# qope/SIPP

Measured on AMD Instinct MI355X. Metric: SIPP proof-gen wall-clock + pairings-aggregated/sec, n=128 (the 3 STARK sub-proofs, hardened G1/G2 AIRs; outer plonky2 proof not included), higher is better.
Workload: dtype u64; 1 GPU; n=128 SIPP instance per GPU: G1ExpStark 127 IO (N=2^16, W+P+Q=1176), G2ExpStark 127 IO (N=2^16, 2314), Fq12ExpStark 14 IO (N=2^13, 7970); IO records on host -> 3 flat proofs on host, the 3 sub-proofs on 3 concurrent HIP streams; parallelism=1 independent SIPP instance(s), one per GPU, no collective

## Files before the change

### include/sipp_hip.h

```cpp
#ifndef SIPP_HIP_H
#define SIPP_HIP_H

#include <stddef.h>
#include <stdint.h>

#ifdef __cplusplus
extern "C" {
#endif

typedef struct sipp_ctx sipp_ctx;

typedef enum {
    SIPP_OK = 0,
    SIPP_E_BADARG = -1,
    SIPP_E_HIP = -2,
    SIPP_E_NOMEM = -3,
    SIPP_E_BUFSZ = -4,
    SIPP_E_SUBGROUP = -5,
    SIPP_E_QUOTIENT = -6,
    SIPP_E_UNSUPPORTED = -7,
    SIPP_E_WITNESS = -8,
    SIPP_E_VERIFY = -9
} sipp_status;

// ... 48 lines not shown
void *sipp_stream(sipp_ctx *ctx);

int sipp_g1_exp_prove(sipp_ctx *ctx, const uint32_t *ios, size_t num_io, uint64_t *proof_out, size_t proof_cap,
                      size_t *proof_len);
int sipp_g2_exp_prove(sipp_ctx *ctx, const uint32_t *ios, size_t num_io, uint64_t *proof_out, size_t proof_cap,
                      size_t *proof_len);
int sipp_fq12_exp_prove(sipp_ctx *ctx, const uint32_t *ios, size_t num_io, uint64_t *proof_out, size_t proof_cap,
                        size_t *proof_len);
int sipp_prove(sipp_ctx *ctx, int kind, const uint32_t *ios, size_t num_io, uint64_t *proof_out, size_t proof_cap,
               size_t *proof_len);
int sipp_prove_async(sipp_ctx *ctx, int kind, const uint32_t *ios, size_t num_io, uint64_t *proof_out,
                     size_t proof_cap);
int sipp_wait(sipp_ctx *ctx, size_t *proof_len);
int sipp_instance_prove(sipp_ctx *const ctxs[3], const uint32_t *const ios[3], const size_t num_io[3],
                        uint64_t *const proof_out[3], const size_t proof_cap[3], size_t proof_len[3]);
int sipp_instances_prove(sipp_ctx *const *ctxs, size_t in_flight, size_t count, const uint32_t *const *ios,
                         const size_t *num_io, uint64_t *const *proof_out, const size_t *proof_cap, size_t *proof_len,
                         int *status);
int sipp_io_shard(size_t num_io, uint32_t world, uint32_t rank, size_t *first, size_t *count);
int sipp_exp_outputs(sipp_ctx *ctx, int kind, uint32_t *ios, size_t num_io);
size_t sipp_proof_size(const sipp_ctx *ctx, int kind, size_t num_io);
size_t sipp_workspace_bytes(int kind, size_t num_io);
size_t sipp_workspace_bytes_cfg(int kind, size_t num_io, const sipp_stark_config *cfg);
int sipp_device_memory(int device, size_t *free_bytes, size_t *total_bytes);
int sipp_stark_shape(const sipp_ctx *ctx, int kind, size_t num_io, uint32_t *log_rows, uint32_t *main_cols,
                     uint32_t *perm_cols, uint32_t *quotient_cols);

int sipp_map_to_g2_prove(sipp_ctx *ctx, const uint32_t *ios, size_t num_io, uint64_t *proof_out, size_t proof_cap,
                         size_t *proof_len);
int sipp_pairing_prove(sipp_ctx *ctx, const uint32_t *ios, size_t num_io, uint64_t *proof_out, size_t proof_cap,
                       size_t *proof_len);
int sipp_stark_verify(const uint64_t *proof, size_t len, const sipp_stark_config *cfg, int *reason);

int sipp_map_to_g2(sipp_ctx *ctx, const uint32_t *msgs, size_t n, uint32_t *map_ios, uint32_t *g2_ios, uint32_t *cleared);

int sipp_inner_product(sipp_ctx *ctx, const uint32_t *g1, const uint32_t *g2, size_t n, uint32_t *out);
int sipp_inner_products(sipp_ctx *ctx, const uint32_t *g1, const uint32_t *g2, size_t n, size_t count, uint32_t *out);

size_t sipp_native_proof_words(size_t n);
int sipp_prove_native(sipp_ctx *ctx, const uint32_t *A, const uint32_t *B, size_t n, uint32_t *proof);
int sipp_verify_native(sipp_ctx *ctx, const uint32_t *A, const uint32_t *B, size_t n, const uint32_t *proof,
                       uint32_t *statement, uint32_t *g1_ios, uint32_t *g2_ios, uint32_t *fq12_ios, int *accepted);

#define SIPP_SALT_SIZE 4
#define SIPP_FRI_MAX_ROUNDS 32
typedef struct {
// ... 170 lines not shown
```

### rust_shim/src/ffi.rs

```rust
use std::os::raw::{c_char, c_int, c_void};

#[repr(C)]
pub struct SippCtxOpaque {
    _p: [u8; 0],
}

#[repr(C)]
#[derive(Clone, Copy)]
pub struct SippStarkConfig {
    pub rate_bits: u32,
    pub cap_height: u32,
    pub pow_bits: u32,
    pub arity_bits: u32,
    pub final_poly_bits: u32,
    pub num_queries: u32,
    pub num_challenges: u32,
    pub pow_rule: u32,
    pub fs_rule: u32,
    pub lookup_rule: u32,
}

pub const SIPP_G1_EXP: c_int = 0;
pub const SIPP_G2_EXP: c_int = 1;
pub const SIPP_FQ12_EXP: c_int = 2;
// ... 171 lines not shown
    pub fn sipp_circuit_workspace_bytes(log_n: u32, p: *const SippPlonkParams, fp: *const SippFriParams, c: *const SippPlonkCircuit) -> usize;
    pub fn sipp_circuit_build(ctx: *mut SippCtxOpaque, log_n: u32, p: *const SippPlonkParams, fp: *const SippFriParams, c: *const SippPlonkCircuit,
                              constants_sigmas: *const u64, gens: *const SippPlonkGenerator, n_gens: usize, sched: *const SippPlonkScheduleHost,
                              circuit_digest: *const u64, out: *mut *mut SippCircuitDataOpaque) -> c_int;
    pub fn sipp_circuit_destroy(cd: *mut SippCircuitDataOpaque);
    pub fn sipp_circuit_verifier_data(cd: *const SippCircuitDataOpaque, cap_out: *mut u64, digest_out: *mut u64) -> c_int;
    pub fn sipp_circuit_proof_size(cd: *const SippCircuitDataOpaque, n_public_inputs: u32) -> usize;
    pub fn sipp_circuit_prove(cd: *mut SippCircuitDataOpaque, wires: *const u64, public_inputs: *const u64, n_public_inputs: u32,
                              proof_out: *mut u64, proof_cap: usize, proof_len: *mut usize) -> c_int;
    pub fn sipp_circuit_prove_inputs(cd: *mut SippCircuitDataOpaque, cells: *const u64, values: *const u64, n_inputs: usize,
                                     public_inputs: *const u64, n_public_inputs: u32, proof_out: *mut u64, proof_cap: usize,
                                     proof_len: *mut usize) -> c_int;
    pub fn sipp_circuit_set_input_map(cd: *mut SippCircuitDataOpaque, cells: *const u64, sources: *const u64, n: usize, n_words: usize,
                                      n_extra: usize) -> c_int;
    pub fn sipp_circuit_prove_words(cd: *mut SippCircuitDataOpaque, words: *const u64, n_words: usize, extra: *const u64, n_extra: usize,
                                    public_inputs: *const u64, n_public_inputs: u32, proof_out: *mut u64, proof_cap: usize,
                                    proof_len: *mut usize) -> c_int;
    pub fn sipp_circuit_verify(cd: *const SippCircuitDataOpaque, proof: *const u64, len: usize, reason: *mut c_int) -> c_int;
    pub fn sipp_plonk_verify_gates(proof: *const u64, len: usize, constants_sigmas_cap: *const u64, p: *const SippPlonkParams, fp: *const SippFriParams,
                                   c: *const SippPlonkCircuit, circuit_digest: *const u64, reason: *mut c_int) -> c_int;
    pub fn sipp_proof_size(ctx: *const SippCtxOpaque, kind: c_int, num_io: usize) -> usize;
    pub fn sipp_workspace_bytes(kind: c_int, num_io: usize) -> usize;
    pub fn sipp_workspace_bytes_cfg(kind: c_int, num_io: usize, cfg: *const SippStarkConfig) -> usize;
    pub fn sipp_device_memory(device: c_int, free_bytes: *mut usize, total_bytes: *mut usize) -> c_int;
    pub fn sipp_stark_shape(ctx: *const SippCtxOpaque, kind: c_int, num_io: usize, log_rows: *mut u32, main_cols: *mut u32,
                            perm_cols: *mut u32, quotient_cols: *mut u32) -> c_int;
    pub fn sipp_inner_product(ctx: *mut SippCtxOpaque, g1: *const u32, g2: *const u32, n: usize, out: *mut u32) -> c_int;
    pub fn sipp_inner_products(ctx: *mut SippCtxOpaque, g1: *const u32, g2: *const u32, n: usize, count: usize, out: *mut u32) -> c_int;
    pub fn sipp_native_proof_words(n: usize) -> usize;
    pub fn sipp_prove_native(ctx: *mut SippCtxOpaque, A: *const u32, B: *const u32, n: usize, proof: *mut u32) -> c_int;
    pub fn sipp_verify_native(ctx: *mut SippCtxOpaque, A: *const u32, B: *const u32, n: usize, proof: *const u32, statement: *mut u32,
                              g1_ios: *mut u32, g2_ios: *mut u32, fq12_ios: *mut u32, accepted: *mut c_int) -> c_int;
    pub fn sipp_fri_const_arity(p: *mut SippFriParams, arity_bits: u32, final_poly_bits: u32, degree_bits: u32);
    pub fn sipp_commit_batch_ex(ctx: *mut SippCtxOpaque, d_in: *const u64, from_coeffs: c_int, d_coeffs: *mut u64, d_lde: *mut u64,
                                d_tree: *mut u64, ncols: usize, log_n: u32, rate_bits: u32, cap_height: u32, d_salt: *const u64,
                                n_salt: u32, cap_out: *mut u64) -> c_int;
    pub fn sipp_fri_proof_size(oracles: *const SippOracle, n_oracles: usize, batches: *const SippFriBatch, n_batches: usize, log_n: u32,
                               p: *const SippFriParams) -> usize;
    pub fn sipp_fri_prove_openings(ctx: *mut SippCtxOpaque, oracles: *const SippOracle, n_oracles: usize, batches: *const SippFriBatch,
                                   n_batches: usize, log_n: u32, p: *const SippFriParams, ch: *mut SippChallenger, proof_out: *mut u64,
                                   proof_cap: usize, proof_len: *mut usize) -> c_int;
    pub fn sipp_plonk_num_partial_products(p: *const SippPlonkParams) -> u32;
    pub fn sipp_plonk_zs_partial_products(ctx: *mut SippCtxOpaque, d_wires: *const u64, d_sigmas: *const u64, log_n: u32, p: *const SippPlonkParams,
                                          betas: *const u64, gammas: *const u64, d_out: *mut u64) -> c_int;
    pub fn sipp_plonk_quotient_chunks(ctx: *mut SippCtxOpaque, d_wires_lde: *const u64, d_sigmas_lde: *const u64, d_zs_lde: *const u64, log_n: u32,
                                      rate_bits: u32, p: *const SippPlonkParams, betas: *const u64, gammas: *const u64, alphas: *const u64,
// ... 35 lines not shown
```

### sipp_amd/_lib.py

```python
import ctypes as C
import json
import os

import numpy as np

HERE = os.path.dirname(os.path.abspath(__file__))
SO = os.path.join(HERE, "libsipp_hip.so")

P = 2**64 - 2**32 + 1

STATUS = {
    0: "SIPP_OK", -1: "SIPP_E_BADARG", -2: "SIPP_E_HIP", -3: "SIPP_E_NOMEM", -4: "SIPP_E_BUFSZ",
    -5: "SIPP_E_SUBGROUP", -6: "SIPP_E_QUOTIENT", -7: "SIPP_E_UNSUPPORTED", -8: "SIPP_E_WITNESS", -9: "SIPP_E_VERIFY",
}


class SippError(RuntimeError):
    def __init__(self, code, msg=""):
        super().__init__("%s (%d): %s" % (STATUS.get(code, "?"), code, msg))
        self.code = code


class StarkConfig(C.Structure):
    _fields_ = [(n, C.c_uint32) for n in ("rate_bits", "cap_height", "pow_bits", "arity_bits", "final_poly_bits",
# ... 106 lines not shown
    "sipp_map_to_g2": (C.c_int, [vp, vp, C.c_size_t, vp, vp, vp]),
    "sipp_prove_async": (C.c_int, [vp, C.c_int, vp, C.c_size_t, vp, C.c_size_t]),
    "sipp_wait": (C.c_int, [vp, C.POINTER(C.c_size_t)]),
    "sipp_host_poseidon_permute": (C.c_int, [vp, C.c_size_t, C.c_int]),
    "sipp_instances_prove": (C.c_int, [C.POINTER(vp), C.c_size_t, C.c_size_t, C.POINTER(vp), C.POINTER(C.c_size_t), C.POINTER(vp),
                                       C.POINTER(C.c_size_t), C.POINTER(C.c_size_t), C.POINTER(C.c_int)]),
    "sipp_io_shard": (C.c_int, [C.c_size_t, C.c_uint32, C.c_uint32, C.POINTER(C.c_size_t), C.POINTER(C.c_size_t)]),
    "sipp_instance_prove": (C.c_int, [C.POINTER(vp), C.POINTER(vp), C.POINTER(C.c_size_t), C.POINTER(vp),
                                      C.POINTER(C.c_size_t), C.POINTER(C.c_size_t)]),
    "sipp_exp_outputs": (C.c_int, [vp, C.c_int, vp, C.c_size_t]),
    "sipp_inner_product": (C.c_int, [vp, vp, vp, C.c_size_t, vp]),
    "sipp_inner_products": (C.c_int, [vp, vp, vp, C.c_size_t, C.c_size_t, vp]),
    "sipp_native_proof_words": (C.c_size_t, [C.c_size_t]),
    "sipp_prove_native": (C.c_int, [vp, vp, vp, C.c_size_t, vp]),
    "sipp_verify_native": (C.c_int, [vp, vp, vp, C.c_size_t, vp, vp, vp, vp, vp, C.POINTER(C.c_int)]),
    "sipp_stark_verify": (C.c_int, [u64p, C.c_size_t, C.POINTER(StarkConfig), C.POINTER(C.c_int)]),
    "sipp_fri_verify_openings": (C.c_int, [u64p, C.c_size_t, C.POINTER(u64p), u32p, u32p, C.c_size_t, C.POINTER(FriBatch), C.c_size_t, C.c_uint32,
                                           C.POINTER(FriParams), C.POINTER(Challenger), C.POINTER(C.c_int)]),
    "sipp_plonk_verify_gates": (C.c_int, [u64p, C.c_size_t, u64p, C.POINTER(PlonkParams), C.POINTER(FriParams), C.POINTER(PlonkCircuit), u64p,
                                          C.POINTER(C.c_int)]),
    "sipp_proof_size": (C.c_size_t, [vp, C.c_int, C.c_size_t]),
    "sipp_stark_shape": (C.c_int, [vp, C.c_int, C.c_size_t, u32p, u32p, u32p, u32p]),
    "sipp_workspace_bytes": (C.c_size_t, [C.c_int, C.c_size_t]),
    "sipp_device_memory": (C.c_int, [C.c_int, C.POINTER(C.c_size_t), C.POINTER(C.c_size_t)]),
    "sipp_workspace_bytes_cfg": (C.c_size_t, [C.c_int, C.c_size_t, C.POINTER(StarkConfig)]),
    "sipp_fri_const_arity": (None, [C.POINTER(FriParams), C.c_uint32, C.c_uint32, C.c_uint32]),
    "sipp_commit_batch_ex": (C.c_int, [vp, vp, C.c_int, vp, vp, vp, C.c_size_t, C.c_uint32, C.c_uint32, C.c_uint32, vp, C.c_uint32, vp]),
    "sipp_fri_proof_size": (C.c_size_t, [C.POINTER(Oracle), C.c_size_t, C.POINTER(FriBatch), C.c_size_t, C.c_uint32, C.POINTER(FriParams)]),
    "sipp_fri_prove_openings": (C.c_int, [vp, C.POINTER(Oracle), C.c_size_t, C.POINTER(FriBatch), C.c_size_t, C.c_uint32,
                                          C.POINTER(FriParams), C.POINTER(Challenger), vp, C.c_size_t, C.POINTER(C.c_size_t)]),
    "sipp_plonk_num_partial_products": (C.c_uint32, [C.POINTER(PlonkParams)]),
    "sipp_plonk_zs_partial_products": (C.c_int, [vp, vp, vp, C.c_uint32, C.POINTER(PlonkParams), u64p, u64p, vp]),
    "sipp_plonk_quotient_chunks": (C.c_int, [vp, vp, vp, vp, C.c_uint32, C.c_uint32, C.POINTER(PlonkParams), u64p, u64p, u64p, vp]),
    "sipp_plonk_quotient_chunks_ex": (C.c_int, [vp, vp, vp, vp, C.c_uint32, C.c_uint32, C.POINTER(PlonkParams), u64p, u64p, u64p, vp, C.c_uint32, vp]),
    "sipp_plonk_prove_ex": (C.c_int, [vp, vp, vp, C.POINTER(Oracle), u64p, C.POINTER(Oracle), C.c_uint32, C.POINTER(PlonkParams), C.POINTER(FriParams),
                                      u64p, u64p, C.c_uint32, vp, C.c_uint32, vp, C.c_size_t, C.POINTER(C.c_size_t)]),
    "sipp_plonk_perm_proof_size": (C.c_size_t, [C.c_uint32, C.POINTER(PlonkParams), C.POINTER(FriParams)]),
    "sipp_plonk_gates_proof_size": (C.c_size_t, [C.c_uint32, C.POINTER(PlonkParams), C.POINTER(FriParams), C.POINTER(PlonkCircuit), C.c_uint32]),
    "sipp_plonk_prove_gates": (C.c_int, [vp, vp, vp, C.POINTER(Oracle), u64p, C.POINTER(Oracle), C.c_uint32, C.POINTER(PlonkParams), C.POINTER(FriParams),
                                         C.POINTER(PlonkCircuit), u64p, u64p, C.c_uint32, vp, C.c_size_t, C.POINTER(C.c_size_t)]),
    "sipp_plonk_generate_witness": (C.c_int, [vp, vp, vp, C.c_uint32, C.c_uint32, C.c_uint32, C.POINTER(PlonkGenerator), C.c_size_t, u64p]),
    "sipp_plonk_generate_witness_levels": (C.c_int, [vp, vp, vp, C.c_uint32, C.c_uint32, C.c_uint32, C.POINTER(PlonkGenerator), C.c_size_t, u64p,
                                                     C.POINTER(PlonkSchedule)]),
    "sipp_circuit_workspace_bytes": (C.c_size_t, [C.c_uint32, C.POINTER(PlonkParams), C.POINTER(FriParams), C.POINTER(PlonkCircuit)]),
    "sipp_circuit_build": (C.c_int, [vp, C.c_uint32, C.POINTER(PlonkParams), C.POINTER(FriParams), C.POINTER(PlonkCircuit), vp, C.POINTER(PlonkGenerator),
                                     C.c_size_t, C.POINTER(PlonkScheduleHost), u64p, C.POINTER(vp)]),
# ... 626 lines not shown
```

### sipp_amd/csrc/prover.hip

```cpp
#include <map>

#include "ctx.hpp"
#include "prover.hpp"

namespace {

using gl::E2;

template <bool REV>
__device__ __forceinline__ uint64_t block_scan_mul_256(uint64_t v, uint64_t* s) {
    const int t = REV ? 255 - (int)threadIdx.x : (int)threadIdx.x;
    s[t] = v;
    __syncthreads();
    for (int off = 1; off < 256; off <<= 1) {
        uint64_t o = t >= off ? s[t - off] : 1;
        __syncthreads();
        v = gl::mul(v, o);
        s[t] = v;
        __syncthreads();
    }
    return v;
}

__device__ __forceinline__ void block_scan4_mul_256(uint64_t (&v)[4], uint64_t (*s)[256]) {
// ... 117 lines not shown
        ulonglong2 v = z[k];
        v.x = gl::mul(tb, v.x);
        v.y = gl::mul(tb, v.y);
        z[k] = v;
    }
}

struct QuotArgs {
    const uint64_t* lde;
    const uint64_t* zlde;
    const uint64_t* aux;
    const int64_t* prog;
    int prog_len;
    int W, nm, nc, cbase, tbits;
    uint32_t log_n, log_m;
    size_t lde_stride;
    uint64_t alpha[2], beta[2], gamma[2];
    const uint32_t* seg_off;
    const uint32_t* seg_cnt;
    const uint64_t* seg_pow;
    const uint32_t* apoly3;
    int n_seg;
    uint64_t* part;
    const uint64_t* per_tab[AIR_N_PERIODIC];
    uint32_t per_mask[AIR_N_PERIODIC];
    const uint64_t* vper_tab;
    uint32_t vper_mask;
    uint64_t zh_inv[2];
    uint64_t zh[2];
    uint64_t ninv;
    uint64_t g_inv;
    uint64_t w_m;
    uint32_t p_limbs[16];
    uint64_t* out;
    int K;
    const uint32_t* apow3;
    uint64_t alphaK[2];
    uint32_t ginv3[2][8][3];
    uint64_t gamma_inv[2], alpha16[2];
    int chunks;
    uint64_t* rest_part;
};

struct QCtx {
    const uint64_t* lde;
    size_t lde_stride;
    uint64_t alpha0, alpha1;
    size_t j, jn, m;
    uint64_t p0, p1, p2, p3, p4, p5, p6, p7, p8, p9, p10, p11;
    uint64_t acc0, acc1;
    const uint64_t* vper;
    uint32_t vper_stride;
    __device__ __forceinline__ uint64_t periodic(int k) const {
        static_assert(AIR_N_PERIODIC == 12, "periodic(): update the select chain");
        if (k >= AIR_N_PERIODIC) return vper[(size_t)(k - AIR_N_PERIODIC) * vper_stride];
        if (k < 4) return k == 0 ? p0 : k == 1 ? p1 : k == 2 ? p2 : p3;
        if (k < 8) return k == 4 ? p4 : k == 5 ? p5 : k == 6 ? p6 : p7;
        return k == 8 ? p8 : k == 9 ? p9 : k == 10 ? p10 : p11;
    }
    __device__ __forceinline__ uint64_t local(int c) const { return lde[(size_t)c * lde_stride + j]; }
    __device__ __forceinline__ uint64_t next(int c) const { return lde[(size_t)c * lde_stride + jn]; }
    __device__ __forceinline__ void emit(uint64_t v) {
        acc0 = gl::mad(acc0, alpha0, v);
        acc1 = gl::mad(acc1, alpha1, v);
    }
};

template <int N>
__device__ __forceinline__ int qvec(const int64_t* w, const QCtx& c, uint64_t (&out)[N]) {
    const int nt = (int)w[1];
#pragma unroll
    for (int i = 0; i < N; i++) out[i] = 0;
    for (int t = 0; t < nt; t++) {
        const int64_t* tm = w + 2 + 5 * t;
        const int cbase = (int)tm[1], stride = (int)tm[2], flag = (int)tm[3], neg = (int)tm[4];
        uint64_t f = gl::from_i64(tm[0]);
        if (flag >= 0) {
            uint64_t pv = c.periodic(flag);
            if (neg) pv = gl::sub(1, pv);
            f = gl::mul(f, pv);
        }
        uint64_t v[N];
#pragma unroll
        for (int i = 0; i < N; i++) v[i] = c.local(cbase + i * stride);
#pragma unroll
        for (int i = 0; i < N; i++) out[i] = gl::mad(f, v[i], out[i]);
    }
    return 2 + 5 * nt;
}

template <bool POLY>
__global__ void __launch_bounds__(64) quotient_prog_kernel(QuotArgs a, int seg0) {
    const size_t m = (size_t)1 << a.log_m;
    const size_t j = (size_t)blockIdx.x * 64 + threadIdx.x;
    const int g = seg0 + (int)blockIdx.y;
    const uint32_t i = gl::bitrev((uint32_t)j, a.log_m);
    QCtx c;
    c.lde = a.lde;
    c.lde_stride = a.lde_stride;
    c.alpha0 = a.alpha[0];
    c.alpha1 = a.alpha[1];
    c.m = m;
    c.j = j;
    c.jn = gl::bitrev((uint32_t)((i + 2) & (m - 1)), a.log_m);
    c.acc0 = c.acc1 = 0;
    c.vper = a.vper_tab + (i & a.vper_mask);
    c.vper_stride = a.vper_mask + 1;
#define SIPP_PER(k) c.p##k = a.per_tab[k][i & a.per_mask[k]]
    SIPP_PER(0); SIPP_PER(1); SIPP_PER(2); SIPP_PER(3); SIPP_PER(4); SIPP_PER(5);
    SIPP_PER(6); SIPP_PER(7); SIPP_PER(8); SIPP_PER(9); SIPP_PER(10); SIPP_PER(11);
#undef SIPP_PER
    const int64_t* w = a.prog + a.seg_off[g];
    const uint32_t n_poly = a.seg_cnt[g];
    if (POLY) {
        gl::Acc6 f0, f1;
        f0.zero();
        f1.zero();
        const uint64_t* __restrict__ lde = a.lde;
        const uint64_t* __restrict__ aux = a.aux;
        const size_t stride = a.lde_stride, jl = c.j, jn = c.jn;
        const uint64_t p0 = c.p0, p1 = c.p1, p2 = c.p2, p3 = c.p3, p4 = c.p4, p5 = c.p5, p6 = c.p6, p7 = c.p7, p8 = c.p8, p9 = c.p9,
                       p10 = c.p10, p11 = c.p11;
        const uint64_t* __restrict__ vper = c.vper;
        const uint32_t vper_stride = c.vper_stride;
        auto periodic = [&](int k) -> uint64_t {
            static_assert(AIR_N_PERIODIC == 12, "periodic(): update the select chain");
            if (k >= AIR_N_PERIODIC) return vper[(size_t)(k - AIR_N_PERIODIC) * vper_stride];
            if (k < 4) return k == 0 ? p0 : k == 1 ? p1 : k == 2 ? p2 : p3;
            if (k < 8) return k == 4 ? p4 : k == 5 ? p5 : k == 6 ? p6 : p7;
            return k == 8 ? p8 : k == 9 ? p9 : k == 10 ? p10 : p11;
        };
        auto operand = [&](int kind, int idx) -> uint64_t {
            return kind == 0 ? lde[(size_t)idx * stride + jl] : kind == 1 ? lde[(size_t)idx * stride + jn] : kind == 2 ? aux[(size_t)idx * m + jl]
                                                                                                                  : periodic(idx);
        };
        for (uint32_t op = 0; op < n_poly; op++) {
            const int nmono = (int)w[1];
            w += 2;
            uint64_t sum = 0;
            for (int mo = 0; mo < nmono; mo++) {
                const int64_t coef = *w++;
                const int nf = (int)*w++;
                if (nf == 0) {
                    sum = gl::add(sum, gl::from_i64(coef));
                    continue;
                }
                uint64_t t = operand((int)w[0], (int)w[1]);
                w += 2;
                for (int f = 1; f < nf; f++) {
                    t = gl::mul(t, operand((int)w[0], (int)w[1]));
                    w += 2;
                }
                if (coef == 1) sum = gl::add(sum, t);
                else if (coef == -1) sum = gl::sub(sum, t);
                else sum = gl::mad(gl::from_i64(coef), t, sum);
            }
            const uint32_t* __restrict__ pw = a.apoly3 + 3 * (n_poly - 1 - op);
            f0.mac((uint32_t)sum, (uint32_t)(sum >> 32), pw);
            f1.mac((uint32_t)sum, (uint32_t)(sum >> 32), pw + 192);
        }
        c.acc0 = f0.reduce();
        c.acc1 = f1.reduce();
    } else {
        const int sign_col = (int)w[1], cbase = (int)w[2], ncl = (int)w[3], lb = (int)w[4];
        const int64_t coffset = w[5];
        const int grp = (int)w[6];
        w += 7;
        const int64_t* qdesc = w;
        w += 2 + 5 * (int)w[1];
        uint64_t e[32];
#pragma unroll
        for (int k = 0; k < 32; k++) e[k] = 0;
        uint64_t psum[2] = {0, 0};
        const int np = (int)*w++;
        const uint32_t n_slices = (n_poly >> 31) ? (n_poly >> 8) & 0xffu : 1u, slice = (n_poly >> 31) ? n_poly & 0xffu : 0u;
        for (int p = 0; p < np; p++) {
            if (n_slices > 1 && (uint32_t)p % n_slices != slice) {
                w += 1;
                w += 2 + 5 * (int)w[1];
                w += 2 + 5 * (int)w[1];
                continue;
            }
            const uint64_t coef = gl::from_i64(*w++);
            uint64_t va[16], vb[16];
            w += qvec<16>(w, c, va);
            w += qvec<16>(w, c, vb);
#pragma unroll
            for (int ch = 0; ch < 2; ch++) {
                gl::Acc6 Ae, Ao, Be, Bo;
                Ae.zero(); Ao.zero(); Be.zero(); Bo.zero();
#pragma unroll
                for (int i = 0; i < 8; i++) {
                    const uint32_t* g3 = a.ginv3[ch][i];
                    Ae.mac((uint32_t)va[2 * i], (uint32_t)(va[2 * i] >> 32), g3);
                    Ao.mac((uint32_t)va[2 * i + 1], (uint32_t)(va[2 * i + 1] >> 32), g3);
                    Be.mac((uint32_t)vb[2 * i], (uint32_t)(vb[2 * i] >> 32), g3);
                    Bo.mac((uint32_t)vb[2 * i + 1], (uint32_t)(vb[2 * i + 1] >> 32), g3);
                }
                const uint64_t ae = Ae.reduce(), ao = Ao.reduce(), be = Be.reduce(), bo = Bo.reduce();
                const uint64_t cross = gl::add(gl::mul(ae, bo), gl::mul(ao, be));
                uint64_t t = gl::mad(gl::mul(ao, bo), a.gamma_inv[ch], gl::mul(ae, be));
                t = gl::mad(cross, 65536, t);
                psum[ch] = gl::mad(coef, t, psum[ch]);
            }
        }
        const int nl = slice == 0 ? (int)*w++ : 0;
        for (int p = 0; p < nl; p++) {
            const uint64_t coef = gl::from_i64(*w++);
            uint64_t va[16];
            w += qvec<16>(w, c, va);
#pragma unroll
            for (int ii = 0; ii < 16; ii++) e[ii] = gl::mad(coef, va[ii], e[ii]);
        }
        if (slice == 0) {
        uint64_t q[17];
        (void)qvec<17>(qdesc, c, q);
        const uint64_t s = c.local(sign_col);
        const uint64_t sgn = gl::sub(1, gl::add(s, s));
        uint64_t cprev = 0;
        const uint64_t coff = gl::from_i64(coffset);
        uint64_t d[32];
#pragma unroll
        for (int k = 0; k < 32; k++) {
            uint64_t al = 0, ah = 0;
#pragma unroll
            for (int ii = 0; ii < 17; ii++) {
                const int jj = k - ii;
                if (jj >= 0 && jj < 16) {
                    al += (uint64_t)(uint32_t)q[ii] * a.p_limbs[jj];
                    ah += (uint64_t)(uint32_t)(q[ii] >> 32) * a.p_limbs[jj];
                }
            }
            const uint64_t l = al + (ah << 32);
            const uint32_t h = (uint32_t)(ah >> 32) + (l < al ? 1u : 0u);
            const uint64_t qp = gl::reduce96(h, l);
            d[k] = gl::sub(e[k], gl::mul(sgn, qp));
        }
        const uint64_t wgt = (uint64_t)1 << (16 * grp);
#pragma unroll
        for (int mm = 0; mm < 32; mm++) {
            if (mm < 32 / grp) {
                uint64_t v;
                if (grp == 2) v = gl::mad(d[(2 * mm + 1) & 31], 65536, d[(2 * mm) & 31]);
                else v = d[mm];
                uint64_t ck = 0;
                if (mm < 32 / grp - 1) {
                    for (int l = 0; l < ncl; l++)
                        ck = gl::mad(c.local(cbase + mm * ncl + l), (uint64_t)1 << (lb * l), ck);
                    ck = gl::sub(ck, coff);
                }
                v = gl::sub(v, cprev);
                v = gl::mad(ck, wgt, v);
                c.emit(v);
                cprev = ck;
            }
        }
        c.emit(gl::mul(s, gl::sub(s, 1)));
        }
        c.acc0 = gl::mad(a.alpha16[0], psum[0], c.acc0);
        c.acc1 = gl::mad(a.alpha16[1], psum[1], c.acc1);
    }
    a.part[((size_t)g * 2 + 0) * m + j] = gl::mul(c.acc0, a.seg_pow[2 * g]);
    a.part[((size_t)g * 2 + 1) * m + j] = gl::mul(c.acc1, a.seg_pow[2 * g + 1]);
}

__global__ void alpha_pow3_kernel(uint64_t a0, uint64_t a1, int K, int nc, uint32_t* __restrict__ out) {
    const int t = blockIdx.x * blockDim.x + threadIdx.x;
    const int total = 2 * 3 + nc * 2 * 6;
    if (t >= total) return;
    int c, e;
    if (t < 6) {
        c = t / 3;
        e = K - 1 - t % 3;
    } else {
        const int k = (t - 6) / 12, r = (t - 6) % 12, slot = r % 6;
        c = r / 6;
        e = K - 1 - (3 + 2 * k) - (slot >> 1) * 2 * nc - (slot & 1);
    }
    uint32_t l[3];
    gl::limbs3(l, gl::pow(c ? a1 : a0, (uint64_t)e));
    for (int q = 0; q < 3; q++) out[3 * t + q] = l[q];
}

// ... 579 lines not shown
    uint64_t* totals = arena_alloc_t<uint64_t>(ctx, (size_t)2 * P * nblk);
    if (!totals) return SIPP_E_NOMEM;
    {
        ProfScope ps(ctx, "z_phase_a");
        if (zr == 8)
            hipLaunchKernelGGL(z_phase_a<8>, dim3(nblk, P / 2), dim3(256), 0, ctx->stream, d_trace, n, a->n_main, a->n_checked,
                               a->checked_base, gamma[0], gamma[1], beta[0], beta[1], d_zv, totals);
        else
            hipLaunchKernelGGL(z_phase_a<4>, dim3(nblk, P / 2), dim3(256), 0, ctx->stream, d_trace, n, a->n_main, a->n_checked,
                               a->checked_base, gamma[0], gamma[1], beta[0], beta[1], d_zv, totals);
    }
    {
        ProfScope ps(ctx, "z_phase_bc");
        hipLaunchKernelGGL(z_phase_b, dim3(P), dim3(256), 0, ctx->stream, totals, (int)nblk);
        if (zr == 8)
            hipLaunchKernelGGL(z_phase_c<8>, dim3(nblk, P), dim3(256), 0, ctx->stream, d_zv, n, totals);
        else
            hipLaunchKernelGGL(z_phase_c<4>, dim3(nblk, P), dim3(256), 0, ctx->stream, d_zv, n, totals);
    }
    SIPP_CHECK_HIP(ctx, hipGetLastError());
    return SIPP_OK;
}

int sipp_k_quotient(sipp_ctx* ctx, const air_spec_t* a, uint32_t log_n, const uint64_t* d_lde, const uint64_t* d_zlde,
                    size_t lde_stride, const uint64_t* d_aux, const uint64_t alpha[2], const uint64_t beta[2],
                    const uint64_t gamma[2], uint64_t* d_out) {
    const uint32_t log_m = log_n + 1;
    const size_t n = (size_t)1 << log_n, m = (size_t)1 << log_m;
    QuotArgs q{};
    q.lde = d_lde; q.zlde = d_zlde; q.aux = d_aux; q.lde_stride = lde_stride;
    q.prog = sipp_air_prog_device(ctx, a);
    if (!q.prog) return SIPP_E_HIP;
    q.prog_len = a->prog_len;
    q.W = a->n_main + 2 * a->n_checked; q.nm = a->n_main; q.nc = a->n_checked; q.cbase = a->checked_base;
    q.tbits = a->table_bits; q.log_n = log_n; q.log_m = log_m;
    q.alpha[0] = alpha[0]; q.alpha[1] = alpha[1]; q.gamma[0] = gamma[0]; q.gamma[1] = gamma[1];
    q.beta[0] = beta[0]; q.beta[1] = beta[1];
    const uint64_t g = gl::root_of_unity(log_n), wm = gl::root_of_unity(log_m);
    for (int k = 0; k < AIR_N_PERIODIC; k++) {
        const uint64_t mk = (uint64_t)AIR_PERIODIC[k][0], r0 = (uint64_t)AIR_PERIODIC[k][1];
        uint64_t* t = sipp_table_get(ctx, 200 + k, log_n, 0);
        if (!t) {
            const uint64_t K = n / mk;
            std::vector<uint64_t> v(2 * mk);
            const uint64_t gs = gl::inv(gl::pow(g, r0)), scale = gl::mul(K % gl::P, gl::inv(n % gl::P));
            for (uint64_t i = 0; i < 2 * mk; i++) {
                uint64_t x = gl::mul(gl::GEN, gl::pow(wm, i));
                uint64_t y = gl::mul(x, gs);
                uint64_t num = gl::sub(gl::pow(y, n), 1), den = gl::sub(gl::pow(y, K), 1);
                v[i] = gl::mul(gl::mul(num, gl::inv(den)), scale);
            }
            SIPP_TRY(sipp_table_put(ctx, 200 + k, log_n, 0, v, &t));
        }
        q.per_tab[k] = t;
        q.per_mask[k] = (uint32_t)(2 * mk - 1);
    }
    q.vper_tab = nullptr;
    q.vper_mask = 0;
    if (a->n_vflag + a->n_vconst > 0) {
        const uint32_t lr = (uint32_t)a->log_rows;
        const size_t R = (size_t)1 << lr, R2 = 2 * R;
        const int nv = a->n_vflag + a->n_vconst;
        uint64_t* t = sipp_table_get(ctx, 104, log_n, (uint64_t)a->kind);
        if (!t) {
            std::vector<uint64_t> tab((size_t)nv * R2), col(R2);
            const uint64_t shift = gl::pow(gl::GEN, (uint64_t)1 << (log_n - lr));
            std::map<std::vector<int64_t>, int> seen;
            std::vector<int64_t> vals(R);
            for (int k = 0; k < nv; k++) {
                for (size_t r = 0; r < R; r++) vals[r] = air_vper_value(a, k, (int)r);
                auto it = seen.find(vals);
                if (it != seen.end()) {
                    memcpy(&tab[(size_t)k * R2], &tab[(size_t)it->second * R2], R2 * 8);
                    continue;
                }
                seen.emplace(vals, k);
                for (size_t r = 0; r < R; r++) col[r] = gl::from_i64(vals[r]);
                sipp_host_ntt(col.data(), lr, true);
// ... 19 lines not shown
    q.ninv = gl::inv(n % gl::P);
    q.g_inv = gl::inv(g);
    q.w_m = wm;
    for (int i = 0; i < 16; i++) q.p_limbs[i] = AIR_BN_P_LIMBS[i];
    q.out = d_out;
    for (int ch = 0; ch < 2; ch++) {
        if (alpha[ch] == 0) return sipp_fail(ctx, SIPP_E_UNSUPPORTED, "quotient: a zero constraint challenge");
        const uint64_t gi = gl::inv(alpha[ch]);
        q.gamma_inv[ch] = gi;
        q.alpha16[ch] = gl::pow(alpha[ch], 16);
        uint64_t x = 1;
        for (int i = 0; i < 8; i++) {
            gl::limbs3(q.ginv3[ch][i], x);
            x = gl::mul(x, gi);
        }
    }
    int n_gadget_segs = 0;
    ArenaScope scope(ctx);
    {
        std::vector<uint32_t> off, cnt;
        std::vector<int> ncons;
        const int64_t* w = a->prog;
        const int64_t* end = a->prog + a->prog_len;
        while (w < end && w[0] == 1) {
            off.push_back((uint32_t)(w - a->prog));
            cnt.push_back(0);
            if (w[6] != 2) return sipp_fail(ctx, SIPP_E_UNSUPPORTED, "quotient: gadgets must pair their limbs (group 2)");
            ncons.push_back(32 / (int)w[6] + 1);
            w += 7;
            w += 2 + 5 * w[1];
            int64_t np = *w++;
            for (int64_t p = 0; p < np; p++) {
                w += 1;
                w += 2 + 5 * w[1];
                w += 2 + 5 * w[1];
            }
            int64_t nl = *w++;
            for (int64_t p = 0; p < nl; p++) {
                w += 1;
                w += 2 + 5 * w[1];
            }
            if (np > 64) {
                const uint32_t nsl = (uint32_t)std::min<int64_t>(SIPP_QUOTIENT_MAX_SLICES, (np + 39) / 40);
                cnt.back() = 0x80000000u | (nsl << 8);
                for (uint32_t k = 1; k < nsl; k++) {
                    off.push_back(off.back());
                    cnt.push_back(0x80000000u | (nsl << 8) | k);
                    ncons.push_back(0);
                }
            }
        }
        while (w < end) {
            off.push_back((uint32_t)(w - a->prog));
            uint32_t k = 0;
            while (w < end && k < 64) {
                int64_t nmono = w[1];
                w += 2;
                for (int64_t mo = 0; mo < nmono; mo++) w += 2 + 2 * w[1];
                k++;
            }
            cnt.push_back(k);
            ncons.push_back((int)k);
        }
        const int ns = (int)off.size();
        q.n_seg = ns;
        n_gadget_segs = 0;
        auto is_gadget = [](uint32_t c) { return c == 0 || (c >> 31) != 0; };
        while (n_gadget_segs < ns && is_gadget(cnt[n_gadget_segs])) n_gadget_segs++;
        for (int g = n_gadget_segs; g < ns; g++)
            if (is_gadget(cnt[g])) return sipp_fail(ctx, SIPP_E_UNSUPPORTED, "quotient: gadgets must precede the polynomial constraints");
        std::vector<uint64_t> host((size_t)ns * 2 + ns + 2 + 192, 0);
        int after = 0;
        for (int g = ns - 1; g >= 0; g--) {
            host[2 * g] = gl::pow(alpha[0], (uint64_t)after);
// ... 200 lines not shown
```

Measured before the change: 2494 pairings/s.

## Use lazy reduction and run-batched integer sums in quotient gadget evaluation

Restructures the quotient kernel's limb-vector evaluation so that consecutive terms sharing a periodic flag are accumulated as 32-bit-split integer sums with one 96-bit reduction per run. It also switches many Goldilocks mul/mad/add calls to non-canonicalizing variants and special-cases coefficients of ±1. The aim is to cut modular reductions in the hot quotient loop. Periodic columns move from twelve per-thread registers into a single packed table indexed on demand, which lowers register pressure but adds loads. A host-side program walker validates coefficient and carry bounds so the lazy sums cannot overflow, and is exposed through new API entry points.

```diff
diff --git a/include/sipp_hip.h b/include/sipp_hip.h
--- a/include/sipp_hip.h
+++ b/include/sipp_hip.h
@@ -94,6 +94,8 @@
 size_t sipp_proof_size(const sipp_ctx *ctx, int kind, size_t num_io);
 size_t sipp_workspace_bytes(int kind, size_t num_io);
 size_t sipp_workspace_bytes_cfg(int kind, size_t num_io, const sipp_stark_config *cfg);
+int sipp_quotient_bounds(const int64_t *prog, size_t prog_len, uint64_t *stats);
+int sipp_air_program(int index, const int64_t **prog, size_t *prog_len, int *kind, int *table_bits, int *hardened);
 int sipp_device_memory(int device, size_t *free_bytes, size_t *total_bytes);
 int sipp_stark_shape(const sipp_ctx *ctx, int kind, size_t num_io, uint32_t *log_rows, uint32_t *main_cols,
                      uint32_t *perm_cols, uint32_t *quotient_cols);
diff --git a/rust_shim/src/ffi.rs b/rust_shim/src/ffi.rs
--- a/rust_shim/src/ffi.rs
+++ b/rust_shim/src/ffi.rs
@@ -217,6 +217,9 @@
     pub fn sipp_proof_size(ctx: *const SippCtxOpaque, kind: c_int, num_io: usize) -> usize;
     pub fn sipp_workspace_bytes(kind: c_int, num_io: usize) -> usize;
     pub fn sipp_workspace_bytes_cfg(kind: c_int, num_io: usize, cfg: *const SippStarkConfig) -> usize;
+    pub fn sipp_quotient_bounds(prog: *const i64, prog_len: usize, stats: *mut u64) -> c_int;
+    pub fn sipp_air_program(index: c_int, prog: *mut *const i64, prog_len: *mut usize, kind: *mut c_int, table_bits: *mut c_int,
+                            hardened: *mut c_int) -> c_int;
     pub fn sipp_device_memory(device: c_int, free_bytes: *mut usize, total_bytes: *mut usize) -> c_int;
     pub fn sipp_stark_shape(ctx: *const SippCtxOpaque, kind: c_int, num_io: usize, log_rows: *mut u32, main_cols: *mut u32,
                             perm_cols: *mut u32, quotient_cols: *mut u32) -> c_int;
diff --git a/sipp_amd/_lib.py b/sipp_amd/_lib.py
--- a/sipp_amd/_lib.py
+++ b/sipp_amd/_lib.py
@@ -152,6 +152,8 @@
     "sipp_proof_size": (C.c_size_t, [vp, C.c_int, C.c_size_t]),
     "sipp_stark_shape": (C.c_int, [vp, C.c_int, C.c_size_t, u32p, u32p, u32p, u32p]),
     "sipp_workspace_bytes": (C.c_size_t, [C.c_int, C.c_size_t]),
+    "sipp_quotient_bounds": (C.c_int, [vp, C.c_size_t, u64p]),
+    "sipp_air_program": (C.c_int, [C.c_int, C.POINTER(vp), C.POINTER(C.c_size_t), C.POINTER(C.c_int), C.POINTER(C.c_int), C.POINTER(C.c_int)]),
     "sipp_device_memory": (C.c_int, [C.c_int, C.POINTER(C.c_size_t), C.POINTER(C.c_size_t)]),
     "sipp_workspace_bytes_cfg": (C.c_size_t, [C.c_int, C.c_size_t, C.POINTER(StarkConfig)]),
     "sipp_fri_const_arity": (None, [C.POINTER(FriParams), C.c_uint32, C.c_uint32, C.c_uint32]),
diff --git a/sipp_amd/csrc/prover.hip b/sipp_amd/csrc/prover.hip
--- a/sipp_amd/csrc/prover.hip
+++ b/sipp_amd/csrc/prover.hip
@@ -163,8 +163,7 @@
     const uint32_t* apoly3;
     int n_seg;
     uint64_t* part;
-    const uint64_t* per_tab[AIR_N_PERIODIC];
-    uint32_t per_mask[AIR_N_PERIODIC];
+    const uint64_t* per_all;
     const uint64_t* vper_tab;
     uint32_t vper_mask;
     uint64_t zh_inv[2];
@@ -183,49 +182,95 @@
     uint64_t* rest_part;
 };
 
+__device__ __forceinline__ uint64_t periodic_at(int k, uint32_t i, const uint64_t* __restrict__ per_all, const uint64_t* __restrict__ vper,
+                                                uint32_t vper_stride) {
+    if (k >= AIR_N_PERIODIC) return vper[(size_t)(k - AIR_N_PERIODIC) * vper_stride];
+    const uint64_t d = per_all[k];
+    return per_all[(size_t)(d >> 32) + (i & (uint32_t)d)];
+}
+
 struct QCtx {
     const uint64_t* lde;
     size_t lde_stride;
     uint64_t alpha0, alpha1;
     size_t j, jn, m;
-    uint64_t p0, p1, p2, p3, p4, p5, p6, p7, p8, p9, p10, p11;
+    const uint64_t* per_all;
+    uint32_t i;
     uint64_t acc0, acc1;
     const uint64_t* vper;
     uint32_t vper_stride;
-    __device__ __forceinline__ uint64_t periodic(int k) const {
-        static_assert(AIR_N_PERIODIC == 12, "periodic(): update the select chain");
-        if (k >= AIR_N_PERIODIC) return vper[(size_t)(k - AIR_N_PERIODIC) * vper_stride];
-        if (k < 4) return k == 0 ? p0 : k == 1 ? p1 : k == 2 ? p2 : p3;
-        if (k < 8) return k == 4 ? p4 : k == 5 ? p5 : k == 6 ? p6 : p7;
-        return k == 8 ? p8 : k == 9 ? p9 : k == 10 ? p10 : p11;
-    }
+    __device__ __forceinline__ uint64_t periodic(int k) const { return periodic_at(k, i, per_all, vper, vper_stride); }
     __device__ __forceinline__ uint64_t local(int c) const { return lde[(size_t)c * lde_stride + j]; }
     __device__ __forceinline__ uint64_t next(int c) const { return lde[(size_t)c * lde_stride + jn]; }
     __device__ __forceinline__ void emit(uint64_t v) {
-        acc0 = gl::mad(acc0, alpha0, v);
-        acc1 = gl::mad(acc1, alpha1, v);
+        acc0 = gl::mad_nc(acc0, alpha0, v);
+        acc1 = gl::mad_nc(acc1, alpha1, v);
     }
 };
+
+constexpr uint64_t QVEC_RUN_BOUND = (uint64_t)1 << 31;
 
 template <int N>
 __device__ __forceinline__ int qvec(const int64_t* w, const QCtx& c, uint64_t (&out)[N]) {
     const int nt = (int)w[1];
+    bool first = true;
 #pragma unroll
     for (int i = 0; i < N; i++) out[i] = 0;
-    for (int t = 0; t < nt; t++) {
-        const int64_t* tm = w + 2 + 5 * t;
-        const int cbase = (int)tm[1], stride = (int)tm[2], flag = (int)tm[3], neg = (int)tm[4];
-        uint64_t f = gl::from_i64(tm[0]);
+    for (int t0 = 0; t0 < nt;) {
+        const int64_t* tm = w + 2 + 5 * t0;
+        const int flag = (int)tm[3], neg = flag >= 0 ? (int)tm[4] : 0;
+        int t1 = t0 + 1;
+        while (t1 < nt && (int)w[2 + 5 * t1 + 3] == flag && (flag < 0 || (int)w[2 + 5 * t1 + 4] == neg)) t1++;
+        uint64_t pv = 0;
         if (flag >= 0) {
-            uint64_t pv = c.periodic(flag);
+            pv = c.periodic(flag);
             if (neg) pv = gl::sub(1, pv);
-            f = gl::mul(f, pv);
-        }
-        uint64_t v[N];
-#pragma unroll
-        for (int i = 0; i < N; i++) v[i] = c.local(cbase + i * stride);
-#pragma unroll
-        for (int i = 0; i < N; i++) out[i] = gl::mad(f, v[i], out[i]);
+        }
+        auto take = [=](uint64_t o, uint64_t r) -> uint64_t {
+            if (flag >= 0) return first ? gl::mul_nc(pv, r) : gl::mad_nc(pv, r, o);
+            return first ? r : gl::add_nc(o, gl::canon(r));
+        };
+        if (t1 == t0 + 1 && tm[0] == 1) {
+            const int cbase = (int)tm[1], stride = (int)tm[2];
+            uint64_t v[N];
+#pragma unroll
+            for (int i = 0; i < N; i++) v[i] = c.local(cbase + i * stride);
+#pragma unroll
+            for (int i = 0; i < N; i++) out[i] = take(out[i], v[i]);
+        } else {
+#pragma unroll
+            for (int i0 = 0; i0 < N; i0 += 8) {
+                uint64_t sl[8], sh[8];
+#pragma unroll
+                for (int i = 0; i < 8; i++) sl[i] = sh[i] = 0;
+                for (int t = t0; t < t1; t++) {
+                    const int64_t* u = w + 2 + 5 * t;
+                    const int64_t f = u[0];
+                    const uint32_t mag = (uint32_t)(f < 0 ? 0 - (uint64_t)f : (uint64_t)f);
+                    const int cbase = (int)u[1], stride = (int)u[2];
+                    uint64_t v[8];
+#pragma unroll
+                    for (int i = 0; i < 8; i++)
+                        if (i0 + i < N) v[i] = c.local(cbase + (i0 + i) * stride);
+#pragma unroll
+                    for (int i = 0; i < 8; i++)
+                        if (i0 + i < N) {
+                            const uint64_t x = f < 0 ? gl::P - v[i] : v[i];
+                            sl[i] += (uint64_t)(uint32_t)x * mag;
+                            sh[i] += (uint64_t)(uint32_t)(x >> 32) * mag;
+                        }
+                }
+#pragma unroll
+                for (int i = 0; i < 8; i++)
+                    if (i0 + i < N) {
+                        const uint64_t l = sl[i] + (sh[i] << 32);
+                        const uint32_t h = (uint32_t)(sh[i] >> 32) + (l < sl[i] ? 1u : 0u);
+                        out[i0 + i] = take(out[i0 + i], gl::reduce96_nc(h, l));
+                    }
+            }
+        }
+        first = false;
+        t0 = t1;
     }
     return 2 + 5 * nt;
 }
@@ -247,10 +292,8 @@
     c.acc0 = c.acc1 = 0;
     c.vper = a.vper_tab + (i & a.vper_mask);
     c.vper_stride = a.vper_mask + 1;
-#define SIPP_PER(k) c.p##k = a.per_tab[k][i & a.per_mask[k]]
-    SIPP_PER(0); SIPP_PER(1); SIPP_PER(2); SIPP_PER(3); SIPP_PER(4); SIPP_PER(5);
-    SIPP_PER(6); SIPP_PER(7); SIPP_PER(8); SIPP_PER(9); SIPP_PER(10); SIPP_PER(11);
-#undef SIPP_PER
+    c.per_all = a.per_all;
+    c.i = i;
     const int64_t* w = a.prog + a.seg_off[g];
     const uint32_t n_poly = a.seg_cnt[g];
     if (POLY) {
@@ -260,21 +303,14 @@
         const uint64_t* __restrict__ lde = a.lde;
         const uint64_t* __restrict__ aux = a.aux;
         const size_t stride = a.lde_stride, jl = c.j, jn = c.jn;
-        const uint64_t p0 = c.p0, p1 = c.p1, p2 = c.p2, p3 = c.p3, p4 = c.p4, p5 = c.p5, p6 = c.p6, p7 = c.p7, p8 = c.p8, p9 = c.p9,
-                       p10 = c.p10, p11 = c.p11;
+        const uint64_t* __restrict__ per_all = a.per_all;
         const uint64_t* __restrict__ vper = c.vper;
         const uint32_t vper_stride = c.vper_stride;
-        auto periodic = [&](int k) -> uint64_t {
-            static_assert(AIR_N_PERIODIC == 12, "periodic(): update the select chain");
-            if (k >= AIR_N_PERIODIC) return vper[(size_t)(k - AIR_N_PERIODIC) * vper_stride];
-            if (k < 4) return k == 0 ? p0 : k == 1 ? p1 : k == 2 ? p2 : p3;
-            if (k < 8) return k == 4 ? p4 : k == 5 ? p5 : k == 6 ? p6 : p7;
-            return k == 8 ? p8 : k == 9 ? p9 : k == 10 ? p10 : p11;
-        };
-        auto operand = [&](int kind, int idx) -> uint64_t {
-            return kind == 0 ? lde[(size_t)idx * stride + jl] : kind == 1 ? lde[(size_t)idx * stride + jn] : kind == 2 ? aux[(size_t)idx * m + jl]
-                                                                                                                  : periodic(idx);
-        };
+#define SIPP_OPERAND(kind, idx)                                                                                                   \
+    ((kind) == 0   ? lde[(size_t)(idx) * stride + jl]                                                                                \
+     : (kind) == 1 ? lde[(size_t)(idx) * stride + jn]                                                                                \
+     : (kind) == 2 ? aux[(size_t)(idx) * m + jl]                                                                                     \
+                   : periodic_at((idx), i, per_all, vper, vper_stride))
         for (uint32_t op = 0; op < n_poly; op++) {
             const int nmono = (int)w[1];
             w += 2;
@@ -286,10 +322,11 @@
                     sum = gl::add(sum, gl::from_i64(coef));
                     continue;
                 }
-                uint64_t t = operand((int)w[0], (int)w[1]);
+                uint64_t t = SIPP_OPERAND((int)w[0], (int)w[1]);
                 w += 2;
                 for (int f = 1; f < nf; f++) {
-                    t = gl::mul(t, operand((int)w[0], (int)w[1]));
+                    const uint64_t o = SIPP_OPERAND((int)w[0], (int)w[1]);
+                    t = f + 1 < nf ? gl::mul_nc(t, o) : gl::mul(t, o);
                     w += 2;
                 }
                 if (coef == 1) sum = gl::add(sum, t);
@@ -300,18 +337,15 @@
             f0.mac((uint32_t)sum, (uint32_t)(sum >> 32), pw);
             f1.mac((uint32_t)sum, (uint32_t)(sum >> 32), pw + 192);
         }
+#undef SIPP_OPERAND
         c.acc0 = f0.reduce();
         c.acc1 = f1.reduce();
     } else {
         const int sign_col = (int)w[1], cbase = (int)w[2], ncl = (int)w[3], lb = (int)w[4];
         const int64_t coffset = w[5];
-        const int grp = (int)w[6];
         w += 7;
         const int64_t* qdesc = w;
         w += 2 + 5 * (int)w[1];
-        uint64_t e[32];
-#pragma unroll
-        for (int k = 0; k < 32; k++) e[k] = 0;
         uint64_t psum[2] = {0, 0};
         const int np = (int)*w++;
         const uint32_t n_slices = (n_poly >> 31) ? (n_poly >> 8) & 0xffu : 1u, slice = (n_poly >> 31) ? n_poly & 0xffu : 0u;
@@ -339,67 +373,80 @@
                     Bo.mac((uint32_t)vb[2 * i + 1], (uint32_t)(vb[2 * i + 1] >> 32), g3);
                 }
                 const uint64_t ae = Ae.reduce(), ao = Ao.reduce(), be = Be.reduce(), bo = Bo.reduce();
-                const uint64_t cross = gl::add(gl::mul(ae, bo), gl::mul(ao, be));
-                uint64_t t = gl::mad(gl::mul(ao, bo), a.gamma_inv[ch], gl::mul(ae, be));
-                t = gl::mad(cross, 65536, t);
-                psum[ch] = gl::mad(coef, t, psum[ch]);
-            }
-        }
-        const int nl = slice == 0 ? (int)*w++ : 0;
-        for (int p = 0; p < nl; p++) {
-            const uint64_t coef = gl::from_i64(*w++);
-            uint64_t va[16];
-            w += qvec<16>(w, c, va);
-#pragma unroll
-            for (int ii = 0; ii < 16; ii++) e[ii] = gl::mad(coef, va[ii], e[ii]);
+                const uint64_t cross = gl::mad_nc(ae, bo, gl::mul_nc(ao, be));
+                uint64_t t = gl::mad_nc(gl::mul_nc(ao, bo), a.gamma_inv[ch], gl::mul_nc(ae, be));
+                t = gl::mad_nc(cross, 65536, t);
+                psum[ch] = gl::mad_nc(coef, t, psum[ch]);
+            }
         }
         if (slice == 0) {
-        uint64_t q[17];
-        (void)qvec<17>(qdesc, c, q);
-        const uint64_t s = c.local(sign_col);
-        const uint64_t sgn = gl::sub(1, gl::add(s, s));
-        uint64_t cprev = 0;
-        const uint64_t coff = gl::from_i64(coffset);
-        uint64_t d[32];
-#pragma unroll
-        for (int k = 0; k < 32; k++) {
-            uint64_t al = 0, ah = 0;
-#pragma unroll
-            for (int ii = 0; ii < 17; ii++) {
-                const int jj = k - ii;
-                if (jj >= 0 && jj < 16) {
-                    al += (uint64_t)(uint32_t)q[ii] * a.p_limbs[jj];
-                    ah += (uint64_t)(uint32_t)(q[ii] >> 32) * a.p_limbs[jj];
+            uint64_t e[16];
+#pragma unroll
+            for (int k = 0; k < 16; k++) e[k] = 0;
+            const int nl = (int)*w++;
+            for (int p = 0; p < nl; p++) {
+                const int64_t icoef = *w++;
+                uint64_t va[16];
+                w += qvec<16>(w, c, va);
+                if (icoef == 1) {
+#pragma unroll
+                    for (int ii = 0; ii < 16; ii++) e[ii] = gl::add_nc(e[ii], gl::canon(va[ii]));
+                } else if (icoef == -1) {
+#pragma unroll
+                    for (int ii = 0; ii < 16; ii++) e[ii] = gl::add_nc(e[ii], gl::neg(gl::canon(va[ii])));
+                } else {
+                    const uint64_t coef = gl::from_i64(icoef);
+#pragma unroll
+                    for (int ii = 0; ii < 16; ii++) e[ii] = gl::mad_nc(coef, va[ii], e[ii]);
                 }
             }
-            const uint64_t l = al + (ah << 32);
-            const uint32_t h = (uint32_t)(ah >> 32) + (l < al ? 1u : 0u);
-            const uint64_t qp = gl::reduce96(h, l);
-            d[k] = gl::sub(e[k], gl::mul(sgn, qp));
-        }
-        const uint64_t wgt = (uint64_t)1 << (16 * grp);
-#pragma unroll
-        for (int mm = 0; mm < 32; mm++) {
-            if (mm < 32 / grp) {
-                uint64_t v;
-                if (grp == 2) v = gl::mad(d[(2 * mm + 1) & 31], 65536, d[(2 * mm) & 31]);
-                else v = d[mm];
+            uint64_t q[17];
+            (void)qvec<17>(qdesc, c, q);
+            const uint64_t s = c.local(sign_col);
+            const uint64_t sgn = gl::sub(1, gl::add(s, s));
+            uint64_t cprev = 0;
+            const uint64_t coff = gl::from_i64(coffset);
+            uint64_t d[32];
+#pragma unroll
+            for (int k = 0; k < 32; k++) {
+                uint64_t al = 0, ah = 0;
+#pragma unroll
+                for (int ii = 0; ii < 17; ii++) {
+                    const int jj = k - ii;
+                    if (jj >= 0 && jj < 16) {
+                        al += (uint64_t)(uint32_t)q[ii] * a.p_limbs[jj];
+                        ah += (uint64_t)(uint32_t)(q[ii] >> 32) * a.p_limbs[jj];
+                    }
+                }
+                const uint64_t l = al + (ah << 32);
+                const uint32_t h = (uint32_t)(ah >> 32) + (l < al ? 1u : 0u);
+                const uint64_t qp = gl::reduce96_nc(h, l);
+                d[k] = gl::sub(k < 16 ? gl::canon(e[k]) : 0, gl::mul(sgn, qp));
+            }
+#pragma unroll
+            for (int mm = 0; mm < 16; mm++) {
+                uint64_t v = gl::mad(d[2 * mm + 1], 65536, d[2 * mm]);
                 uint64_t ck = 0;
-                if (mm < 32 / grp - 1) {
-                    for (int l = 0; l < ncl; l++)
-                        ck = gl::mad(c.local(cbase + mm * ncl + l), (uint64_t)1 << (lb * l), ck);
-                    ck = gl::sub(ck, coff);
+                if (mm < 15) {
+                    uint64_t cl = 0, chh = 0;
+                    for (int l = 0; l < ncl; l++) {
+                        const uint64_t x = c.local(cbase + mm * ncl + l);
+                        const uint32_t wl = 1u << (lb * l);
+                        cl += (uint64_t)(uint32_t)x * wl;
+                        chh += (uint64_t)(uint32_t)(x >> 32) * wl;
+                    }
+                    const uint64_t l64 = cl + (chh << 32);
+                    const uint32_t h = (uint32_t)(chh >> 32) + (l64 < cl ? 1u : 0u);
+                    ck = gl::sub(gl::reduce96(h, l64), coff);
                 }
                 v = gl::sub(v, cprev);
-                v = gl::mad(ck, wgt, v);
-                c.emit(v);
+                c.emit(gl::mad_nc(ck, (uint64_t)1 << 32, v));
                 cprev = ck;
             }
-        }
-        c.emit(gl::mul(s, gl::sub(s, 1)));
-        }
-        c.acc0 = gl::mad(a.alpha16[0], psum[0], c.acc0);
-        c.acc1 = gl::mad(a.alpha16[1], psum[1], c.acc1);
+            c.emit(gl::mul(s, gl::sub(s, 1)));
+        }
+        c.acc0 = gl::mad_nc(a.alpha16[0], psum[0], c.acc0);
+        c.acc1 = gl::mad_nc(a.alpha16[1], psum[1], c.acc1);
     }
     a.part[((size_t)g * 2 + 0) * m + j] = gl::mul(c.acc0, a.seg_pow[2 * g]);
     a.part[((size_t)g * 2 + 1) * m + j] = gl::mul(c.acc1, a.seg_pow[2 * g + 1]);
@@ -1025,6 +1072,98 @@
     return SIPP_OK;
 }
 
+namespace {
+struct GadgetWalk {
+    const int64_t* w;
+    const int64_t* end;
+    struct {
+        uint64_t gadgets, vectors, max_terms, max_run_sum, max_carry_sum;
+    } b{};
+    const char* why = nullptr;
+    bool need(int64_t words) {
+        if (words < 0 || words > end - w) why = "the program ends inside a gadget";
+        return !why;
+    }
+    static uint64_t mag(int64_t f) { return f < 0 ? 0 - (uint64_t)f : (uint64_t)f; }
+    bool vec() {
+        if (!need(2)) return false;
+        const int64_t nt = w[1];
+        if (nt < 0 || nt > (end - w) / 5) why = "the program ends inside a gadget";
+        if (why || !need(2 + 5 * nt)) return false;
+        b.vectors++;
+        b.max_terms = std::max<uint64_t>(b.max_terms, (uint64_t)nt);
+        for (int64_t t0 = 0; t0 < nt;) {
+            const int64_t* tm = w + 2 + 5 * t0;
+            const int64_t flag = tm[3], neg = flag >= 0 ? tm[4] : 0;
+            uint64_t sum = 0;
+            int64_t t1 = t0;
+            while (t1 < nt && (t1 == t0 || (w[2 + 5 * t1 + 3] == flag && (flag < 0 || w[2 + 5 * t1 + 4] == neg)))) {
+                const uint64_t m = mag(w[2 + 5 * t1]);
+                if (m >= QVEC_RUN_BOUND) why = "quotient: a limb vector's coefficient is beyond the lazy sum's range";
+                sum += m < QVEC_RUN_BOUND ? m : QVEC_RUN_BOUND;
+                t1++;
+            }
+            b.max_run_sum = std::max(b.max_run_sum, sum);
+            if (sum >= QVEC_RUN_BOUND) why = "quotient: a run of limb vector terms is beyond the lazy sum's range";
+            t0 = t1;
+        }
+        w += 2 + 5 * nt;
+        return !why;
+    }
+    bool gadget(int64_t* n_products) {
+        if (!need(7)) return false;
+        if (w[6] != 2) why = "quotient: gadgets must pair their limbs (group 2)";
+        const int64_t ncl = w[3], lb = w[4];
+        uint64_t cw = 0;
+        if (ncl < 0 || ncl > 32 || lb < 0 || lb > 30 || (ncl > 1 && lb * (ncl - 1) > 30)) why = "quotient: a carry's shift weights are beyond the lazy sum's range";
+        else
+            for (int64_t l = 0; l < ncl; l++) cw += (uint64_t)1 << (lb * l);
+        b.max_carry_sum = std::max(b.max_carry_sum, cw);
+        if (cw >= QVEC_RUN_BOUND) why = "quotient: a carry's shift weights are beyond the lazy sum's range";
+        if (why) return false;
+        b.gadgets++;
+        w += 7;
+        if (!vec() || !need(1)) return false;
+        const int64_t np = *w++;
+        for (int64_t p = 0; p < np; p++) {
+            if (!need(1)) return false;
+            w += 1;
+            if (!vec() || !vec()) return false;
+        }
+        if (!need(1)) return false;
+        const int64_t nl = *w++;
+        for (int64_t p = 0; p < nl; p++) {
+            if (!need(1)) return false;
+            w += 1;
+            if (!vec()) return false;
+        }
+        *n_products = np;
+        return true;
+    }
+};
+}
+
+extern "C" int sipp_quotient_bounds(const int64_t* prog, size_t prog_len, uint64_t* stats) {
+    if (!prog || !stats) return SIPP_E_BADARG;
+    GadgetWalk g{prog, prog + prog_len};
+    int64_t np;
+    while (g.w < g.end && g.w[0] == 1 && g.gadget(&np)) {}
+    stats[0] = g.b.gadgets; stats[1] = g.b.vectors; stats[2] = g.b.max_terms; stats[3] = g.b.max_run_sum; stats[4] = g.b.max_carry_sum;
+    stats[5] = QVEC_RUN_BOUND;
+    return g.why ? SIPP_E_UNSUPPORTED : SIPP_OK;
+}
+
+extern "C" int sipp_air_program(int index, const int64_t** prog, size_t* prog_len, int* kind, int* table_bits, int* hardened) {
+    if (index < 0 || (size_t)index >= sizeof(AIR_AIRS) / sizeof(AIR_AIRS[0]) || !prog || !prog_len) return SIPP_E_BADARG;
+    const air_spec_t* a = &AIR_AIRS[index];
+    *prog = a->prog;
+    *prog_len = (size_t)a->prog_len;
+    if (kind) *kind = a->kind;
+    if (table_bits) *table_bits = a->table_bits;
+    if (hardened) *hardened = a->hardened;
+    return SIPP_OK;
+}
+
 int sipp_k_quotient(sipp_ctx* ctx, const air_spec_t* a, uint32_t log_n, const uint64_t* d_lde, const uint64_t* d_zlde,
                     size_t lde_stride, const uint64_t* d_aux, const uint64_t alpha[2], const uint64_t beta[2],
                     const uint64_t gamma[2], uint64_t* d_out) {
@@ -1040,23 +1179,25 @@
     q.alpha[0] = alpha[0]; q.alpha[1] = alpha[1]; q.gamma[0] = gamma[0]; q.gamma[1] = gamma[1];
     q.beta[0] = beta[0]; q.beta[1] = beta[1];
     const uint64_t g = gl::root_of_unity(log_n), wm = gl::root_of_unity(log_m);
-    for (int k = 0; k < AIR_N_PERIODIC; k++) {
-        const uint64_t mk = (uint64_t)AIR_PERIODIC[k][0], r0 = (uint64_t)AIR_PERIODIC[k][1];
-        uint64_t* t = sipp_table_get(ctx, 200 + k, log_n, 0);
+    {
+        uint64_t* t = sipp_table_get(ctx, 200, log_n, 0);
         if (!t) {
-            const uint64_t K = n / mk;
-            std::vector<uint64_t> v(2 * mk);
-            const uint64_t gs = gl::inv(gl::pow(g, r0)), scale = gl::mul(K % gl::P, gl::inv(n % gl::P));
-            for (uint64_t i = 0; i < 2 * mk; i++) {
-                uint64_t x = gl::mul(gl::GEN, gl::pow(wm, i));
-                uint64_t y = gl::mul(x, gs);
-                uint64_t num = gl::sub(gl::pow(y, n), 1), den = gl::sub(gl::pow(y, K), 1);
-                v[i] = gl::mul(gl::mul(num, gl::inv(den)), scale);
-            }
-            SIPP_TRY(sipp_table_put(ctx, 200 + k, log_n, 0, v, &t));
-        }
-        q.per_tab[k] = t;
-        q.per_mask[k] = (uint32_t)(2 * mk - 1);
+            std::vector<uint64_t> v(AIR_N_PERIODIC);
+            for (int k = 0; k < AIR_N_PERIODIC; k++) {
+                const uint64_t mk = (uint64_t)AIR_PERIODIC[k][0], r0 = (uint64_t)AIR_PERIODIC[k][1];
+                const uint64_t K = n / mk, at = v.size();
+                v[k] = (at << 32) | (2 * mk - 1);
+                const uint64_t gs = gl::inv(gl::pow(g, r0)), scale = gl::mul(K % gl::P, gl::inv(n % gl::P));
+                for (uint64_t i = 0; i < 2 * mk; i++) {
+                    uint64_t x = gl::mul(gl::GEN, gl::pow(wm, i));
+                    uint64_t y = gl::mul(x, gs);
+                    uint64_t num = gl::sub(gl::pow(y, n), 1), den = gl::sub(gl::pow(y, K), 1);
+                    v.push_back(gl::mul(gl::mul(num, gl::inv(den)), scale));
+                }
+            }
+            SIPP_TRY(sipp_table_put(ctx, 200, log_n, 0, v, &t));
+        }
+        q.per_all = t;
     }
     q.vper_tab = nullptr;
     q.vper_mask = 0;
@@ -1122,24 +1263,13 @@
         std::vector<int> ncons;
         const int64_t* w = a->prog;
         const int64_t* end = a->prog + a->prog_len;
-        while (w < end && w[0] == 1) {
-            off.push_back((uint32_t)(w - a->prog));
+        GadgetWalk gw{w, end};
+        while (gw.w < end && gw.w[0] == 1) {
+            off.push_back((uint32_t)(gw.w - a->prog));
             cnt.push_back(0);
-            if (w[6] != 2) return sipp_fail(ctx, SIPP_E_UNSUPPORTED, "quotient: gadgets must pair their limbs (group 2)");
-            ncons.push_back(32 / (int)w[6] + 1);
-            w += 7;
-            w += 2 + 5 * w[1];
-            int64_t np = *w++;
-            for (int64_t p = 0; p < np; p++) {
-                w += 1;
-                w += 2 + 5 * w[1];
-                w += 2 + 5 * w[1];
-            }
-            int64_t nl = *w++;
-            for (int64_t p = 0; p < nl; p++) {
-                w += 1;
-                w += 2 + 5 * w[1];
-            }
+            int64_t np;
+            if (!gw.gadget(&np)) return sipp_fail(ctx, SIPP_E_UNSUPPORTED, gw.why);
+            ncons.push_back(32 / 2 + 1);
             if (np > 64) {
                 const uint32_t nsl = (uint32_t)std::min<int64_t>(SIPP_QUOTIENT_MAX_SLICES, (np + 39) / 40);
                 cnt.back() = 0x80000000u | (nsl << 8);
@@ -1150,6 +1280,7 @@
                 }
             }
         }
+        w = gw.w;
         while (w < end) {
             off.push_back((uint32_t)(w - a->prog));
             uint32_t k = 0;
```

Measured after the change: 2511 pairings/s, median of 6. No clear change (+0.7%).
